# lianqi1008/Control-GIC

Hardware: AMD Instinct MI355X
Metric: encode+decode MPixels/s at fixed granularity ratio; bpp match vs reference (higher is better)
Workload: dtype f32; 1 GPU; batch 64 of 256x256 per GPU per step, codebook 1024x4, ratio (0.1,0.8,0.1), hot path only (entropy maps + router + VQ + Huffman/mask coder, encode+decode); conv encoder/decoder out of scope, latent synthetic; inputs=8 distinct resident batches in rotation (416 MiB > 256 MiB Infinity Cache)

## Files before the change

control-gic_amd/csrc/cgic_decode.hip:

```cpp
#include "cgic_coder_dev.h"

#include <atomic>

namespace cgic {

constexpr int kWinBytes = 8192;
constexpr int kWinWords = kWinBytes / 4 + 4;

struct WaveDecoder {
    const TableDev &t;
    const uint32_t *lut;
    uint32_t *win;
    const uint8_t *in;
    int nbytes;
    int wb;

    __device__ __forceinline__ void fill(int first_byte)
    {
        const int lane = lane_id();
        wb = first_byte & ~3;
        const uintptr_t g = reinterpret_cast<uintptr_t>(in) + (uintptr_t)wb;
        const uint32_t *ga = reinterpret_cast<const uint32_t *>(g & ~(uintptr_t)3);
        wsh = (int)(g & 3);
        const int limit = (nbytes - wb + wsh + 3) / 4 + 2;
// ... 572 lines not shown
        if (n0 <= 0) a.dcount[b * 3] = n0 == 0 ? -1 : -2;
        if (n1 <= 0) a.dcount[b * 3 + 1] = n1 == 0 ? -1 : -2;
        if (n2 <= 0) a.dcount[b * 3 + 2] = n2 == 0 ? -1 : -2;
    }
    if (s < 0) return;
    const int64_t n_c = (a.h >> 2) * (a.w >> 2), n_m = (a.h >> 1) * (a.w >> 1), n_f = a.h * a.w;
    const int64_t off = s == 0 ? 0 : (s == 1 ? n_c : n_c + n_m);
    const int cap = (int)(s == 0 ? n_c : (s == 1 ? n_m : n_f));
    int32_t *dc = a.dcount + b * 3 + s;
    const uint8_t *in = in0 + s * a.slot;
    const int nb = s == 0 ? n0 : s == 1 ? n1 : n2;
    const int s_pad = s == 0 ? pad0 : s == 1 ? pad1 : pad2;
    __syncthreads();
    uint16_t *dst = a.dsym + b * (n_c + n_m + n_f) + off;
    auto put = [&](int k, int sym) { dst[k] = (uint16_t)sym; };
    FastTables *ft = reinterpret_cast<FastTables *>(reinterpret_cast<int32_t *>(seg + 1) + 2 * kLdsTrieNodes);
    if (nparts == 1) {
        int nw = (nb + 15) >> 4;
        nw = nw < 1 ? 1 : (nw > kDecWaves ? kDecWaves : nw);
        if (nb <= kFastChunks * 8)
            decode_segmented<false>(a.tab, lut, win + wave * kSegWinWords, seg, in, nb, s_pad, 0, wave < nw ? nw : 0, wave, cap, put,
                                    &s_count, ft);
        else
            decode_segmented<true>(a.tab, lut, win + wave * kSegWinWords, seg, in, nb, s_pad, 0, wave < nw ? nw : 0, wave, cap, put,
                                   &s_count, ft);
        __syncthreads();
        if (tid == 0) *dc = s_count > cap ? -3 : s_count;
        return;
    }
    PartSync ps{a.bf + (b * 3 + s) * kDecPartsMax * kWave, a.tick + (b * 3 + s) * kTicketStride, s_entry};
    int nbits = s_pad == 0 ? 0 : (nb - 1) * 8 - s_pad;
    nbits = nbits < 0 ? 0 : nbits;
    const int nchunks = (nbits + kWave - 1) / kWave, per_part = (nchunks + nparts - 1) / nparts;
    if (per_part <= kFastChunks) {
        decode_segmented<true>(a.tab, lut, win + wave * kSegWinWords, seg, in, nb, s_pad, 0, kDecWaves, wave, cap, put, &s_count, ft,
                               part, nparts, 0, 0, nullptr, &ps);
    } else {
        decode_segmented<false>(a.tab, lut, win + wave * kSegWinWords, seg, in, nb, s_pad, 0, kDecWaves, wave, 0,
                                [](int, int) {}, &s_count, (FastTables *)nullptr, part, nparts, 0, 0, s_fn);
        __syncthreads();
        if (wave == 0) part_exchange(part, nparts, s_fn[tid], ps);
        if (tid == 0) s_count = 0;
        __syncthreads();
        decode_segmented<true>(a.tab, lut, win + wave * kSegWinWords, seg, in, nb, s_pad, 0, kDecWaves, wave, cap, put, &s_count, ft,
                               part, nparts, s_entry[0], s_entry[1]);
    }
    __syncthreads();
    if (tid == 0 && part == nparts - 1) *dc = s_count > cap ? -3 : s_count;
}

__global__ __launch_bounds__(kDecThreads) void decode_split_kernel(DecodeArgs a)
{
    decode_split_body(a, own_blk());
}

__global__ __launch_bounds__(kDecThreads) void decode_split_grouped_kernel(Grouped<DecodeArgs> g)
{
    Blk blk;
    decode_split_body(g.a[group_locate(g, &blk)], blk);
}

struct MergeArgs {
    const uint8_t *in;
    int64_t slot;
    const int32_t *nbytes;
    int64_t h, w;
    int mode;
    const uint16_t *dsym;
    const int32_t *dcount;
    int64_t *ind_out;
    int32_t *mc_out, *mm_out, *mf_out;
    const float *codebook;
    int K;
    float *zq;
    const float *codebook2;
    float *zq2;
    int32_t *status;
    int stage_sym, stage_cb;
    int64_t band_syms;
};

__device__ __forceinline__ void wait_decoded(unsigned int *done, unsigned int need, unsigned int total)
{
    if (threadIdx.x == 0) {
        while (__hip_atomic_load(done, __ATOMIC_RELAXED, __HIP_MEMORY_SCOPE_AGENT) < need) __builtin_amdgcn_s_sleep(8);
        const unsigned int old = __hip_atomic_fetch_add(done, 1u, __ATOMIC_RELAXED, __HIP_MEMORY_SCOPE_AGENT);
        if (old + 1u == total) __hip_atomic_store(done, 0u, __ATOMIC_RELAXED, __HIP_MEMORY_SCOPE_AGENT);
        __builtin_amdgcn_fence(__ATOMIC_ACQUIRE, "agent");
    }
    __syncthreads();
}

typedef unsigned int cgic_u32x4 __attribute__((ext_vector_type(4)));
typedef unsigned int cgic_u32x2 __attribute__((ext_vector_type(2)));
__device__ __forceinline__ void nt_store16(void *p, const void *v)
{
    __builtin_nontemporal_store(*reinterpret_cast<const cgic_u32x4 *>(v), reinterpret_cast<cgic_u32x4 *>(p));
}
__device__ __forceinline__ void nt_store8(void *p, const void *v)
{
    __builtin_nontemporal_store(*reinterpret_cast<const cgic_u32x2 *>(v), reinterpret_cast<cgic_u32x2 *>(p));
}

template <int NT, bool WAIT = false>
__device__ __forceinline__ void merge_body(const MergeArgs &a, const Blk blk, unsigned int *done = nullptr, unsigned int need = 0,
                                           unsigned int total = 0)
{
    extern __shared__ __attribute__((aligned(16))) uint32_t sm[];
    __shared__ uint32_t scan_smem[NT / kWave + 1];
    __shared__ int s_status;
    __shared__ int s_hdr[8];
    const int tid = threadIdx.x;
    const int band = blk.x;
    const int64_t b = blk.y;
    const int64_t h = a.h, w = a.w, h2 = h >> 1, w2 = w >> 1, h4 = h >> 2, w4 = w >> 2;
    const int64_t n_c = h4 * w4, n_m = h2 * w2, n_f = h * w;
    const int64_t wc = (n_c + 31) >> 5, wm = (n_m + 31) >> 5;
    const int64_t nsym = n_c + n_m + n_f;
    float4 *cbk = reinterpret_cast<float4 *>(sm);
    uint16_t *lsym = reinterpret_cast<uint16_t *>(cbk + (a.stage_cb ? a.K : 0));
    uint32_t *rawc = reinterpret_cast<uint32_t *>(lsym) + (a.stage_sym ? (nsym + 1) / 2 : 0);
    uint32_t *rawm = rawc + wc + 2;
    uint32_t *mcb = rawm + wm + 2;
    uint32_t *mmb = mcb + wc;
    uint32_t *pcb = mmb + wm;
    uint32_t *pmb = pcb + wc;
    const int mode = a.mode;
    const int64_t nbands = blk.nx;
    const int64_t rows_per = ((h4 + nbands - 1) / nbands) * 4;
    const int64_t r0 = band * rows_per, r1 = r0 + rows_per < h ? r0 + rows_per : h;
    if (r0 >= h) return;
    CGIC_STAMP(10);
    const bool send_mc = mode == 0 || mode == 2 || mode == 3;
    const bool send_mm = mode == 0 || mode == 1;
    const uint8_t *in_mc = a.in + (b * CGIC_NUM_STREAMS + 3) * a.slot;
    const uint8_t *in_mm = a.in + (b * CGIC_NUM_STREAMS + 4) * a.slot;

    if (tid == 0) s_status = 0;
    if (tid < 2) s_hdr[tid] = a.nbytes[b * CGIC_NUM_STREAMS + 3 + tid];
    else if (!WAIT && tid < 5) s_hdr[tid] = a.dcount[b * 3 + (tid - 2)];
    if (send_mc) for (int64_t i = tid; i < wc + 2; i += NT) rawc[i] = reinterpret_cast<const uint32_t *>(in_mc)[i];
    if (send_mm) for (int64_t i = tid; i < wm + 2; i += NT) rawm[i] = reinterpret_cast<const uint32_t *>(in_mm)[i];
    const uint16_t *gsym = a.dsym + b * nsym;
    if (!WAIT && a.stage_sym) {
        const uint32_t *g32 = reinterpret_cast<const uint32_t *>(gsym);
        uint32_t *l32 = reinterpret_cast<uint32_t *>(lsym);
        for (int64_t i = tid; i < (nsym + 1) / 2; i += NT) l32[i] = g32[i];
    }
    if (a.stage_cb && a.zq)
        for (int i = tid; i < a.K; i += NT) cbk[i] = reinterpret_cast<const float4 *>(a.codebook)[i];
    __syncthreads();
    CGIC_STAMP(11);

    if (tid == 0) {
        if (send_mc && (s_hdr[0] != 2 + (n_c >> 3) || (int)(rawc[0] & 0xFF) != 8 - (int)(n_c & 7))) s_status = CGIC_ERR_INVALID;
        if (send_mm && (s_hdr[1] != 2 + (n_m >> 3) || (int)(rawm[0] & 0xFF) != 8 - (int)(n_m & 7))) s_status = CGIC_ERR_INVALID;
    }
    __syncthreads();
    if (s_status) {
        if (WAIT) wait_decoded(done, need, total);
        if (tid == 0 && a.status) atomicMin(&a.status[b], s_status);
        return;
    }
    auto stream_word = [](const uint32_t *raw, int64_t wi, int64_t nbits) -> uint32_t {
        const uint64_t two = (uint64_t)raw[wi] | ((uint64_t)raw[wi + 1] << 32);
        const uint32_t pay = (uint32_t)(two >> 8);
        uint32_t v = __builtin_bswap32(__brev(pay));
        const int64_t rem = nbits - wi * 32;
        if (rem < 32) v &= rem <= 0 ? 0u : ((1u << rem) - 1u);
        return v;
    };
    uint32_t cnt_c, cnt_m;
    __shared__ uint32_t s_cnt[2];
    const bool derived_mm = mode == 3 || mode == 5;
    if (wc <= kWave && wm <= kWave && !derived_mm) {
        const int lane = lane_id(), wave = tid >> 6;
        if (wave < 2) {
            const bool co = wave == 0;
            const int64_t nw_ = co ? wc : wm, nb_ = co ? n_c : n_m;
            uint32_t v = 0;
            if (lane < nw_) {
                if (co ? send_mc : send_mm) v = stream_word(co ? rawc : rawm, lane, nb_);
                else if (co && mode == 4) {
                    v = 0xFFFFFFFFu;
                    const int64_t rem = nb_ - (int64_t)lane * 32;
                    if (rem < 32) v &= (1u << rem) - 1u;
                }
            }
            const uint32_t c = (uint32_t)__popc(v);
            const uint32_t inc = wave_inclusive_scan(c);
            if (lane < nw_) {
                (co ? mcb : mmb)[lane] = v;
                (co ? pcb : pmb)[lane] = inc - c;
            }
            if (lane == kWave - 1) s_cnt[wave] = inc;
        }
        __syncthreads();
        cnt_c = s_cnt[0];
        cnt_m = s_cnt[1];
    } else {
        for (int64_t i = tid; i < wc; i += NT) {
            uint32_t v = 0;
            if (send_mc) v = stream_word(rawc, i, n_c);
            else if (mode == 4) {
                v = 0xFFFFFFFFu;
                const int64_t rem = n_c - i * 32;
                if (rem < 32) v &= (1u << rem) - 1u;
            }
            mcb[i] = v;
        }
        __syncthreads();
        for (int64_t i = tid; i < wm; i += NT) {
            uint32_t v = 0;
            if (send_mm) v = stream_word(rawm, i, n_m);
            else if (mode == 3 || mode == 5) {
                for (int k = 0; k < 32; ++k) {
                    const int64_t j = i * 32 + k;
                    if (j >= n_m) break;
                    bool bit = true;
                    if (mode == 3) {
                        const int64_t y = j / w2, x = j - y * w2, c = (y >> 1) * w4 + (x >> 1);
                        bit = !((mcb[c >> 5] >> (c & 31)) & 1u);
                    }
                    v |= (uint32_t)bit << k;
                }
            }
            mmb[i] = v;
        }
        __syncthreads();
        if (wc <= NT && wm <= NT) {
            __shared__ unsigned long long scan64[NT / kWave + 1];
            const unsigned long long c = ((unsigned long long)(tid < wc ? __popc(mcb[tid]) : 0) << 32) | (unsigned long long)(tid < wm ? __popc(mmb[tid]) : 0);
            unsigned long long tot;
            const unsigned long long ex = block_exclusive_scan(c, scan64, &tot);
            if (tid < wc) pcb[tid] = (uint32_t)(ex >> 32);
            if (tid < wm) pmb[tid] = (uint32_t)ex;
            cnt_c = (uint32_t)(tot >> 32);
            cnt_m = (uint32_t)tot;
            __syncthreads();
        } else {
        uint32_t carry = 0, total;
        for (int64_t base = 0; base < wc; base += NT) {
            const int64_t i = base + tid;
            const uint32_t c = i < wc ? (uint32_t)__popc(mcb[i]) : 0u;
            const uint32_t ex = block_exclusive_scan(c, scan_smem, &total);
            if (i < wc) pcb[i] = carry + ex;
            carry += total;
        }
        cnt_c = carry;
        carry = 0;
        for (int64_t base = 0; base < wm; base += NT) {
            const int64_t i = base + tid;
            const uint32_t c = i < wm ? (uint32_t)__popc(mmb[i]) : 0u;
            const uint32_t ex = block_exclusive_scan(c, scan_smem, &total);
            if (i < wm) pmb[i] = carry + ex;
            carry += total;
        }
        cnt_m = carry;
        __syncthreads();
        }
    }
    CGIC_STAMP(12);

    auto fine_flag = [&](int64_t y, int64_t x, bool *pbc, bool *pbm) -> bool {
        const int64_t j2 = (y >> 1) * w2 + (x >> 1), j4 = (y >> 2) * w4 + (x >> 2);
        const bool bc = (mcb[j4 >> 5] >> (j4 & 31)) & 1u;
        const bool bm = (mmb[j2 >> 5] >> (j2 & 31)) & 1u;
        *pbc = bc; *pbm = bm;
        switch (mode) {
        case 0: return (1 - (int)bm - (int)bc) == 1;
        case 1: return !bm;
        case 2: return !bc;
        case 6: return true;
        default: return false;
        }
    };
    uint32_t fbase = 0;
    {
        uint32_t mine = 0;
        const int wvm = tid >> 6, lnm = tid & 63;
        for (int y2 = wvm; y2 < (int)(r0 >> 1); y2 += NT / 64)
            for (int x2 = lnm; x2 < (int)w2; x2 += 64) {
                bool bc, bm;
                mine += fine_flag(2 * y2, 2 * x2, &bc, &bm) ? 4u : 0u;
            }
        (void)block_exclusive_scan(mine, scan_smem, &fbase);
    }
    CGIC_STAMP(13);
    if (WAIT) {
        wait_decoded(done, need, total);
        if (tid >= 2 && tid < 5) s_hdr[tid] = a.dcount[b * 3 + (tid - 2)];
        if (a.stage_sym) {
            const uint32_t *g32 = reinterpret_cast<const uint32_t *>(gsym);
            uint32_t *l32 = reinterpret_cast<uint32_t *>(lsym);
            for (int64_t i = tid; i < (nsym + 1) / 2; i += NT) l32[i] = g32[i];
        }
        __syncthreads();
    }

    const uint16_t *ds_c = a.stage_sym ? lsym : gsym, *ds_m = ds_c + n_c, *ds_f = ds_m + n_m;
    const int64_t dc_c = s_hdr[2], dc_m = s_hdr[3], dc_f = s_hdr[4];
    uint16_t *bsym = reinterpret_cast<uint16_t *>(pmb + wm);
    int64_t off_c = 0, off_m = 0, off_f = 0;
    if (!a.stage_sym && a.band_syms > 0) {
        auto rank_of = [&](const uint32_t *bits, const uint32_t *pre, int64_t j, int64_t nbits, uint32_t total) -> int64_t {
            if (j >= nbits) return (int64_t)total;
            return (int64_t)pre[j >> 5] + __popc(bits[j >> 5] & ((1u << (j & 31)) - 1u));
        };
        const int64_t c0 = rank_of(mcb, pcb, (r0 >> 2) * w4, n_c, cnt_c), c1 = rank_of(mcb, pcb, (r1 >> 2) * w4, n_c, cnt_c);
        const int64_t m0 = rank_of(mmb, pmb, (r0 >> 1) * w2, n_m, cnt_m), m1 = rank_of(mmb, pmb, (r1 >> 1) * w2, n_m, cnt_m);
        const int64_t f0 = fbase, f1 = f0 + (r1 - r0) * w;
        const int64_t nc = c1 - c0, nm = m1 - m0, nf = (f1 < n_f ? f1 : n_f) - f0;
        if (nc >= 0 && nm >= 0 && nf >= 0 && nc + nm + nf + 3 <= a.band_syms) {
            for (int64_t i = tid; i < nc; i += NT) bsym[i] = ds_c[c0 + i];
            for (int64_t i = tid; i < nm; i += NT) bsym[nc + i] = ds_m[m0 + i];
            for (int64_t i = tid; i < nf; i += NT) bsym[nc + nm + i] = ds_f[f0 + i];
            __syncthreads();
            off_c = c0; off_m = m0 - nc; off_f = f0 - nc - nm;
            ds_c = bsym; ds_m = bsym; ds_f = bsym;
        }
    }
    const bool has_c = mode == 0 || mode == 2 || mode == 3 || mode == 4;
    const bool has_m = mode == 0 || mode == 1 || mode == 3 || mode == 5;
    const bool has_f = mode == 0 || mode == 1 || mode == 2 || mode == 6;
    int st = 0;
    if (dc_c == -3 || dc_m == -3 || dc_f == -3) st = CGIC_ERR_INVALID;
    if (has_c && dc_c >= 0 && dc_c != cnt_c) st = CGIC_ERR_INVALID;
    if (has_m && dc_m >= 0 && dc_m != cnt_m) st = CGIC_ERR_INVALID;
    const bool use_c = has_c && dc_c >= 0, use_m = has_m && dc_m >= 0, use_f = has_f && dc_f >= 0;

    int64_t *ind_out = a.ind_out ? a.ind_out + b * n_f : nullptr;
    float *zq = a.zq ? a.zq + b * 4 * n_f : nullptr;
    float *zq2 = a.zq2 ? a.zq2 + b * 4 * n_f : nullptr;
    uint32_t fcarry = fbase;
    int bad_index = 0;
    const int w4i = (int)w4;
    for (int64_t qbase = r0 * w4; qbase < r1 * w4; qbase += NT) {
        const int64_t q = qbase + tid;
        const bool live = q < r1 * w4;
        int64_t v[4] = {0, 0, 0, 0};
        bool bfa = false, bfb = false;
        int y = 0, xq = 0;
        if (live) {
            y = (int)q / w4i; xq = (int)q - y * w4i;
            const int64_t j4 = (int64_t)(y >> 2) * w4 + xq, j2 = (int64_t)(y >> 1) * w2 + 2 * xq;
            bool bc, bma, bmb, dummy;
            bfa = fine_flag(y, 4 * xq, &bc, &bma);
            bfb = fine_flag(y, 4 * xq + 2, &dummy, &bmb);
            bad_index |= (int)(mode == 0 && bc && (bma || bmb));
            int64_t vc = 0, va = 0, vb = 0;
            if (bc && use_c) vc = ds_c[(int64_t)pcb[j4 >> 5] + __popc(mcb[j4 >> 5] & ((1u << (j4 & 31)) - 1u)) - off_c];
            if (use_m) {
                const uint32_t word = mmb[j2 >> 5], below = word & ((1u << (j2 & 31)) - 1u);
                const int64_t rk = (int64_t)pmb[j2 >> 5] + __popc(below) - off_m;
                if (bma) va = ds_m[rk];
                if (bmb) vb = ds_m[rk + (bma ? 1 : 0)];
            }
            v[0] = v[1] = vc + va;
            v[2] = v[3] = vc + vb;
            const int64_t i = (int64_t)y * w + 4 * xq;
            if (a.mc_out && (y & 3) == 0) a.mc_out[b * n_c + j4] = bc;
            if (a.mm_out && (y & 1) == 0) { const int2 t2 = make_int2(bma, bmb); nt_store8(a.mm_out + b * n_m + j2, &t2); }
            if (a.mf_out) { const int4 t4 = make_int4(bfa, bfa, bfb, bfb); nt_store16(a.mf_out + b * n_f + i, &t4); }
        }
        uint32_t ftotal;
        uint32_t frank = block_exclusive_scan((bfa ? 2u : 0u) + (bfb ? 2u : 0u), scan_smem, &ftotal) + fcarry;
        if (live) {
            if (bfa) {
                if (use_f) {
                    if ((int64_t)frank < dc_f) v[0] += ds_f[(int64_t)frank - off_f];
                    if ((int64_t)frank + 1 < dc_f) v[1] += ds_f[(int64_t)frank + 1 - off_f];
                }
                frank += 2;
            }
            if (bfb && use_f) {
                if ((int64_t)frank < dc_f) v[2] += ds_f[(int64_t)frank - off_f];
                if ((int64_t)frank + 1 < dc_f) v[3] += ds_f[(int64_t)frank + 1 - off_f];
            }
            const int64_t i = (int64_t)y * w + 4 * xq;
            if (ind_out) {
                nt_store16(ind_out + i, &v[0]);
                nt_store16(ind_out + i + 2, &v[2]);
            }
            if (zq || zq2) {
#pragma unroll
                for (int k = 0; k < 4; ++k)
                    if (v[k] < 0 || v[k] >= a.K) { bad_index = 1; v[k] = 0; }
            }
            if (zq) {
                float4 e[4];
#pragma unroll
                for (int k = 0; k < 4; ++k) e[k] = a.stage_cb ? cbk[v[k]] : reinterpret_cast<const float4 *>(a.codebook)[v[k]];
                const float4 o0 = make_float4(e[0].x, e[1].x, e[2].x, e[3].x), o1 = make_float4(e[0].y, e[1].y, e[2].y, e[3].y);
                const float4 o2 = make_float4(e[0].z, e[1].z, e[2].z, e[3].z), o3 = make_float4(e[0].w, e[1].w, e[2].w, e[3].w);
                nt_store16(zq + i, &o0);
                nt_store16(zq + n_f + i, &o1);
                nt_store16(zq + 2 * n_f + i, &o2);
                nt_store16(zq + 3 * n_f + i, &o3);
            }
            if (zq2) {
                float4 e[4];
#pragma unroll
                for (int k = 0; k < 4; ++k) e[k] = reinterpret_cast<const float4 *>(a.codebook2)[v[k]];
                *reinterpret_cast<float4 *>(zq2 + i) = make_float4(e[0].x, e[1].x, e[2].x, e[3].x);
                *reinterpret_cast<float4 *>(zq2 + n_f + i) = make_float4(e[0].y, e[1].y, e[2].y, e[3].y);
                *reinterpret_cast<float4 *>(zq2 + 2 * n_f + i) = make_float4(e[0].z, e[1].z, e[2].z, e[3].z);
                *reinterpret_cast<float4 *>(zq2 + 3 * n_f + i) = make_float4(e[0].w, e[1].w, e[2].w, e[3].w);
            }
        }
        fcarry += ftotal;
    }
    CGIC_STAMP(14);
    if (r1 == h && has_f && (dc_f >= 0 ? dc_f != (int64_t)fcarry : fcarry != 0)) st = CGIC_ERR_INVALID;
    if (bad_index) s_status = CGIC_ERR_INVALID;
    __syncthreads();
    if (tid == 0 && a.status && (st || s_status)) atomicMin(&a.status[b], st ? st : s_status);
}

template <int NT>
__global__ __launch_bounds__(NT) void merge_kernel(MergeArgs a)
{
    merge_body<NT>(a, own_blk());
}

__global__ __launch_bounds__(kMergeThreads) void merge_grouped_kernel(Grouped<MergeArgs> g)
{
    Blk blk;
    merge_body<kMergeThreads>(g.a[group_locate(g, &blk)], blk);
}

struct DecodeMergeArgs {
// ... 250 lines not shown
```

control-gic_amd/csrc/cgic_decode_ss.hip:

```cpp
#include "cgic_coder_dev.h"

namespace cgic {

constexpr int kSsEnd = 0xFF;

struct SsLayout {
    int nbits[3];
    int c[4];
    int off[3];
};
__device__ __forceinline__ int sel3(int s, int v0, int v1, int v2) { return s == 0 ? v0 : (s == 1 ? v1 : v2); }

__device__ __forceinline__ uint32_t ss_bits(uint32_t d0, uint32_t d1, uint32_t d2, int pos)
{
    const uint32_t hi = pos < 32 ? d0 : d1, lo = pos < 32 ? d1 : d2;
    const uint32_t r = __builtin_amdgcn_alignbit(hi, lo, 32u - ((uint32_t)pos & 31u));
    return (pos & 31) ? r : hi;
}

template <bool WRITE, typename Put>
__device__ __forceinline__ int ss_walk(const TableDev &t, const uint32_t *lut, const uint8_t *stage, const SsLayout &L, int g,
                                       int entry, int *count, Put put)
{
    const int s = (g >= L.c[1]) + (g >= L.c[2]);
// ... 21 lines not shown
        auto step = [&]() {
            const bool go = pos < lim;
            const uint32_t e = *reinterpret_cast<const uint32_t *>(lutb + ((w0 >> ish) & imask));
            const int len = (int)(e & 0xFF);
            const int np = pos + len;
            const bool ok = go && np <= remc;
            if (WRITE) { if (ok) put(s, n, (int)(e >> 8)); }
            const uint32_t r = 32u - (uint32_t)len;
            w0 = __builtin_amdgcn_alignbit(w0, w1, r);
            w1 = __builtin_amdgcn_alignbit(w1, w2, r);
            w2 <<= (len & 31);
            pos = go ? np : pos;
            n += ok ? 1 : 0;
        };
        while (__builtin_amdgcn_ballot_w64(pos < lim) != 0) {
            step();
            step();
        }
        *count = n;
        return (pos < 64 || pos > remc) ? kSsEnd : pos - 64;
    }
    while (pos < 64) {
        if (pos >= rem) { *count = n; return kSsEnd; }
        const uint32_t bits = ss_bits(d0, d1, d2, pos);
        const uint32_t e = lut[bits >> (32 - LB)];
        int len = (int)(e & 0xFF), sym = (int)(e >> 8);
        if (len == 0) {
            if (sym == 0xFFFFFF) { *count = n; return kSsEnd; }
            const unsigned long long w0 = ((unsigned long long)d0 << 32) | d1, w1 = ((unsigned long long)d2 << 32) | d3;
            const unsigned long long win = pos ? (w0 << pos) | (w1 >> (64 - pos)) : w0;
            int node = sym, k = LB;
            sym = -1;
            while (pos + k < rem && k < 64) {
                const int c = t.child[2 * node + (int)((win >> (63 - k)) & 1ull)];
                ++k;
                if (c == INT32_MIN) break;
                if (c < 0) { sym = ~c; break; }
                node = c;
            }
            if (sym < 0) { *count = n; return kSsEnd; }
            len = k;
        }
        if (pos + len > rem) { *count = n; return kSsEnd; }
        if (WRITE) put(s, n, sym);
        pos += len;
        ++n;
    }
    *count = n;
    return pos - 64;
}


constexpr int kSsMaxSweeps = 32;
constexpr int kMeEntries = 15;
constexpr uint32_t kMeEnd = 15;

struct MeFn { uint32_t r[4]; };

__device__ __forceinline__ MeFn me_identity() { return MeFn{{0x03020100u, 0x07060504u, 0x0B0A0908u, 0x0F0E0D0Cu}}; }
__device__ __forceinline__ MeFn me_const0() { return MeFn{{0u, 0u, 0u, 0u}}; }
__device__ __forceinline__ MeFn me_compose(const MeFn &prev, const MeFn &cur)
{
    MeFn o;
#pragma unroll
    for (int k = 0; k < 4; ++k) {
        const uint32_t sel = prev.r[k];
        const uint32_t s7 = sel & 0x07070707u;
        const uint32_t lo = __builtin_amdgcn_perm(cur.r[1], cur.r[0], s7);
        const uint32_t hi = __builtin_amdgcn_perm(cur.r[3], cur.r[2], s7);
        const uint32_t m = ((sel >> 3) & 0x01010101u) * 0xFFu;
        o.r[k] = (hi & m) | (lo & ~m);
    }
    return o;
}
__device__ __forceinline__ uint32_t me_apply(const MeFn &f, uint32_t e)
{
    const uint32_t w = e < 8 ? (e < 4 ? f.r[0] : f.r[1]) : (e < 12 ? f.r[2] : f.r[3]);
    return (w >> (8 * (e & 3))) & 0xFFu;
}
__device__ __forceinline__ MeFn me_shfl_up(const MeFn &f, int d)
{
    MeFn o;
#pragma unroll
    for (int k = 0; k < 4; ++k) o.r[k] = (uint32_t)__shfl_up((int)f.r[k], d, kWave);
    return o;
}
__device__ __forceinline__ MeFn me_wave_scan(MeFn f)
{
    const int lane = lane_id();
#pragma unroll
    for (int d = 1; d < kWave; d <<= 1) {
        const MeFn p = me_shfl_up(f, d);
        const MeFn c = me_compose(p, f);
        if (lane >= d) f = c;
    }
    return f;
}

__device__ __forceinline__ MeFn me_walk_all(const TableDev &t, const uint32_t *lut, const uint8_t *stage, const SsLayout &L, int g,
                                            unsigned long long *cnt_lo, unsigned long long *cnt_hi)
{
    const int s = (g >= L.c[1]) + (g >= L.c[2]);
    const int ch = g - sel3(s, L.c[0], L.c[1], L.c[2]);
    const int rem = sel3(s, L.nbits[0], L.nbits[1], L.nbits[2]) - 64 * ch;
    const uint32_t *q = reinterpret_cast<const uint32_t *>(stage + sel3(s, L.off[0], L.off[1], L.off[2]) + 8 * ch);
    const uint32_t r0 = __builtin_bswap32(q[0]), r1 = __builtin_bswap32(q[1]), r2 = __builtin_bswap32(q[2]), r3 = __builtin_bswap32(q[3]);
    const uint32_t d0 = __builtin_amdgcn_alignbit(r0, r1, 24), d1 = __builtin_amdgcn_alignbit(r1, r2, 24), d2 = __builtin_amdgcn_alignbit(r2, r3, 24);
    const int LB = t.lut_bits;
    const int remc = rem < 128 ? rem : 128, lim = rem < 64 ? rem : 64;
    const uint32_t ish = 30u - (uint32_t)LB, imask = ((1u << LB) - 1u) << 2;
    const char *lutb = reinterpret_cast<const char *>(lut);
    const int E = t.max_len < kMeEntries ? t.max_len : kMeEntries;
    int pos[kMeEntries], n[kMeEntries];
#pragma unroll
    for (int e = 0; e < kMeEntries; ++e) { pos[e] = e < E ? e : 1 << 20; n[e] = 0; }
    for (;;) {
        bool any = false;
#pragma unroll
        for (int e = 0; e < kMeEntries; ++e) any |= pos[e] < lim;
        if (__builtin_amdgcn_ballot_w64(any) == 0) break;
#pragma unroll
        for (int e = 0; e < kMeEntries; ++e) {
            const int p = pos[e];
            const bool go = p < lim;
            const uint32_t bits = ss_bits(d0, d1, d2, p & 63);
            const uint32_t ent = *reinterpret_cast<const uint32_t *>(lutb + ((bits >> ish) & imask));
            const int np = p + (int)(ent & 0xFF);
            const bool ok = go && np <= remc;
            pos[e] = go ? np : p;
            n[e] += ok ? 1 : 0;
        }
    }
    MeFn f;
    unsigned long long lo = 0, hi = 0;
#pragma unroll
    for (int k = 0; k < 4; ++k) f.r[k] = 0;
#pragma unroll
    for (int e = 0; e < kMeEntries; ++e) {
        const int p = pos[e];
        const uint32_t x = (e >= E || p < 64 || p > remc) ? kMeEnd : (uint32_t)(p - 64);
        f.r[e >> 2] |= x << (8 * (e & 3));
        if (e < 8) lo |= (unsigned long long)(uint32_t)n[e] << (8 * e);
        else hi |= (unsigned long long)(uint32_t)n[e] << (8 * (e - 8));
    }
    f.r[3] |= kMeEnd << 24;
    *cnt_lo = lo; *cnt_hi = hi;
    return f;
}

__device__ __forceinline__ void decode_image_body(const DecodeArgs &a, const int stage_cap, const int chunk_cap, const Blk blk)
{
    extern __shared__ __attribute__((aligned(16))) uint32_t sm[];
    __shared__ int s_scan[kDecWaves + 1];
    __shared__ int s_base[4];
    __shared__ MeFn s_fn[kDecWaves];
    uint32_t *lut = sm;
    uint8_t *stage = reinterpret_cast<uint8_t *>(lut + (1 << a.tab.lut_bits));
    uint8_t *ent = stage + stage_cap, *ext = ent + chunk_cap, *cnt = ext + chunk_cap;
    const int tid = threadIdx.x, T = blockDim.x, lane = lane_id(), wave = tid >> 6, nw = T >> 6;
    const int64_t b = blk.x;
    CGIC_STAMP3(0);
    const uint8_t *in0 = a.in + (b * CGIC_NUM_STREAMS) * a.slot;
    int nb[3];
#pragma unroll
    for (int s = 0; s < 3; ++s) nb[s] = (a.stream_mask >> s & 1) ? a.nbytes[b * CGIC_NUM_STREAMS + s] : -2;
    const int pad[3] = {in0[0], in0[a.slot], in0[2 * a.slot]};
    {
        const uint4 *gl = reinterpret_cast<const uint4 *>(a.tab.lut);
        uint4 *dl = reinterpret_cast<uint4 *>(lut);
        const int n4 = (1 << a.tab.lut_bits) >> 2;
        const bool mark = a.tab.max_len <= a.tab.lut_bits;
        auto fix = [mark](uint32_t e) { return mark && (e & 0xFFu) == 0u ? e | 0xFFu : e; };
        if (n4 == 0 && tid < (1 << a.tab.lut_bits)) lut[tid] = fix(a.tab.lut[tid]);
        for (int base = 0; base < n4; base += 8 * T) {
            uint4 v[8];
#pragma unroll
            for (int k = 0; k < 8; ++k) {
                const int i = base + k * T + tid;
                v[k] = i < n4 ? gl[i] : uint4{0u, 0u, 0u, 0u};
            }
#pragma unroll
            for (int k = 0; k < 8; ++k) {
                const int i = base + k * T + tid;
                if (i < n4) dl[i] = uint4{fix(v[k].x), fix(v[k].y), fix(v[k].z), fix(v[k].w)};
            }
        }
    }
    const int64_t n_c = (a.h >> 2) * (a.w >> 2), n_m = (a.h >> 1) * (a.w >> 1), n_f = a.h * a.w;
    const int cap[3] = {(int)n_c, (int)n_m, (int)n_f};
    SsLayout L;
    int stage_used = 0;
    bool fits = true;
    L.c[0] = 0;
#pragma unroll
    for (int s = 0; s < 3; ++s) {
        if (nb[s] > a.slot) nb[s] = (int)a.slot;
        int bits = nb[s] <= 0 || pad[s] == 0 ? 0 : (nb[s] - 1) * 8 - pad[s];
        bits = bits < 0 ? 0 : bits;
        L.nbits[s] = bits;
        L.c[s + 1] = L.c[s] + ((bits + 63) >> 6);
        L.off[s] = stage_used;
        stage_used += bits ? (((bits + 7) >> 3) + 1 + 24 + 15) & ~15 : 0;
    }
    const int C = L.c[3];
    if (stage_used > stage_cap || C > chunk_cap) fits = false;
    if (tid == 0) {
        if (a.status) a.status[b] = 0;
#pragma unroll
        for (int s = 0; s < 3; ++s) {
            if (nb[s] <= 0) a.dcount[b * 3 + s] = nb[s] == 0 ? -1 : -2;
            else if (!fits) a.dcount[b * 3 + s] = -3;
        }
    }
    if (!fits) return;
    CGIC_STAMP3(1);
#pragma unroll
    for (int s = 0; s < 3; ++s) {
        if (!L.nbits[s]) continue;
        const int words = ((((L.nbits[s] + 7) >> 3) + 1 + 24 + 15) & ~15) >> 4;
        const uint4 *g = reinterpret_cast<const uint4 *>(in0 + s * a.slot);
        uint4 *d = reinterpret_cast<uint4 *>(stage + L.off[s]);
        const int lim = (int)(a.slot >> 4);
        for (int i = tid; i < words; i += T) d[i] = i < lim ? g[i] : uint4{0u, 0u, 0u, 0u};
    }
    __syncthreads();
    CGIC_STAMP3(2);
    const int R = (C + T - 1) / T;
    const int g0 = tid * R < C ? tid * R : C, g1 = g0 + R < C ? g0 + R : C;
    auto is_first = [&](int g) { return g == L.c[0] || g == L.c[1] || g == L.c[2]; };
    auto nop = [](int, int, int) {};
    int dbg_sweeps = 0;
    const bool all_entries = a.tab.max_len <= a.tab.lut_bits && a.tab.max_len <= kMeEntries;
    bool stuck = false;
    {
        int prev = 0;
        for (int g = g0; g < g1; ++g) {
            int e = prev;
            if (is_first(g)) e = 0;
            else if (g == g0) {
                const int sg = (g >= L.c[1]) + (g >= L.c[2]);
                const int chg = g - sel3(sg, L.c[0], L.c[1], L.c[2]);
                const int m = (64 * chg) % a.tab.len_gcd;
                e = m ? a.tab.len_gcd - m : 0;
            }
            int n;
            prev = ss_walk<false>(a.tab, lut, stage, L, g, e, &n, nop);
            ent[g] = (uint8_t)e; ext[g] = (uint8_t)prev; cnt[g] = (uint8_t)n;
        }
    }
    __syncthreads();
    CGIC_STAMP3(3);
    for (;;) {
        ++dbg_sweeps;
        int changed = 0;
        for (int g = g0; g < g1; ++g) {
            const int e = is_first(g) ? 0 : ext[g - 1];
            if (e != ent[g]) {
                int n;
                const int x = ss_walk<false>(a.tab, lut, stage, L, g, e, &n, nop);
                ent[g] = (uint8_t)e; ext[g] = (uint8_t)x; cnt[g] = (uint8_t)n;
                changed = 1;
            }
        }
        if (!__syncthreads_or(changed)) break;
        if (all_entries && dbg_sweeps >= kSsMaxSweeps) { stuck = true; break; }
    }
    if (stuck) {
        MeFn mine = me_identity();
        unsigned long long c_lo = 0, c_hi = 0;
        for (int g = g0; g < g1; ++g) {
            MeFn f = me_walk_all(a.tab, lut, stage, L, g, &c_lo, &c_hi);
            if (is_first(g + 1)) f = me_const0();
            mine = me_compose(mine, f);
        }
        const MeFn incl = me_wave_scan(mine);
        if (lane == kWave - 1) s_fn[wave] = incl;
        __syncthreads();
        MeFn before = me_identity();
        for (int w2 = 0; w2 < wave; ++w2) before = me_compose(before, s_fn[w2]);
        MeFn prev = me_shfl_up(incl, 1);
        if (lane == 0) prev = me_identity();
        uint32_t e = me_apply(prev, me_apply(before, 0u));
        if (g0 < g1 && is_first(g0)) e = 0;
        if (R == 1) {
            if (g0 < g1) {
                const unsigned long long cw = e < 8 ? c_lo : c_hi;
                ent[g0] = (uint8_t)(e == kMeEnd ? kSsEnd : (int)e);
                cnt[g0] = e == kMeEnd ? (uint8_t)0 : (uint8_t)((cw >> (8 * (e & 7))) & 0xFFull);
            }
        } else {
            int en = e == kMeEnd ? kSsEnd : (int)e;
            for (int g = g0; g < g1; ++g) {
                if (is_first(g)) en = 0;
                int n;
                const int x = ss_walk<false>(a.tab, lut, stage, L, g, en, &n, nop);
                ent[g] = (uint8_t)en; cnt[g] = (uint8_t)n;
                en = x;
            }
        }
        dbg_sweeps += 1;
        __syncthreads();
    }
    CGIC_STAMP3(4);
    if (a.stats && tid == 0) {
        atomicAdd(&a.stats[0], (unsigned int)dbg_sweeps);
        atomicAdd(&a.stats[1], 1u);
        atomicMax(&a.stats[2], (unsigned int)dbg_sweeps);
    }
#ifdef CGIC_PHASE_CLOCKS
    if (blk.x == 0 && tid == 0) g_phase_clk[9] = dbg_sweeps;
#endif
    int mine = 0;
    for (int g = g0; g < g1; ++g) mine += cnt[g];
    int inc = wave_inclusive_scan(mine);
    if (lane == kWave - 1) s_scan[wave] = inc;
    __syncthreads();
    if (wave == 0) {
        const int v = lane < nw ? s_scan[lane] : 0;
        const int vi = wave_inclusive_scan(v);
        if (lane < nw) s_scan[lane] = vi - v;
        if (lane == nw - 1) s_scan[kDecWaves] = vi;
    }
    __syncthreads();
    int run = s_scan[wave] + inc - mine;
    const int total = s_scan[kDecWaves];
    {
        int r = run;
        for (int g = g0; g < g1; ++g) {
            if (g == L.c[1]) s_base[1] = r;
            if (g == L.c[2]) s_base[2] = r;
            r += cnt[g];
        }
        if (tid == 0) {
            s_base[0] = 0; s_base[3] = total;
            if (L.c[2] == C) s_base[2] = total;
            if (L.c[1] == C) s_base[1] = total;
        }
    }
    __syncthreads();
    CGIC_STAMP3(5);
    uint16_t *dst = a.dsym + b * (n_c + n_m + n_f);
    for (int g = g0; g < g1; ++g) {
        const int s = (g >= L.c[1]) + (g >= L.c[2]);
        const int at = run - s_base[s];
        const int cap_s = sel3(s, cap[0], cap[1], cap[2]);
        uint16_t *dst_s = dst + sel3(s, 0, (int)n_c, (int)(n_c + n_m)) + at;
        int n;
        ss_walk<true>(a.tab, lut, stage, L, g, (int)ent[g], &n,
                      [&](int, int k, int sym) { if (at + k < cap_s) dst_s[k] = (uint16_t)sym; });
        run += n;
    }
    CGIC_STAMP3(6);
    if (tid < 3 && sel3(tid, nb[0], nb[1], nb[2]) > 0) {
        const int n = s_base[tid + 1] - s_base[tid];
        a.dcount[b * 3 + tid] = n > sel3(tid, cap[0], cap[1], cap[2]) ? -3 : n;
    }
}

__global__ __launch_bounds__(kDecThreads) void decode_image_kernel(DecodeArgs a, int stage_cap, int chunk_cap)
{
    decode_image_body(a, stage_cap, chunk_cap, own_blk());
}

__global__ __launch_bounds__(kDecThreads) void decode_image_grouped_kernel(Grouped<DecodeImageArgs> g)
{
    Blk blk;
    const DecodeImageArgs &p = g.a[group_locate(g, &blk)];
    decode_image_body(p.a, p.stage_cap, p.chunk_cap, blk);
}

}

using namespace cgic;
static GroupedRegistrar reg_decode_image(KID_DECODE_IMAGE, [](const GroupRec *const *recs, int n, hipStream_t s) {
    return launch_grouped(decode_image_grouped_kernel, "decode_image_grouped_kernel", recs[0]->block, LDS_ALWAYS, recs, n, s); });
```

Before: 129,100 MPixels/s.

## Resolve self-synchronizing Huffman chunk entries with wave shuffles instead of block sweeps

For one chunk per thread, the decoder now passes chunk exit states between lanes with shuffles. It iterates within each wave until the states converge and publishes only the wave-boundary exit through shared memory, so the number of block-wide barriers and shared-memory round trips drops. The symbol-count scan is rebuilt to need a single barrier: stream bases are computed by every thread from per-wave totals, replacing the extra scan and base passes. The kernel also issues the first LUT and stream-staging global loads early, before the layout checks, to overlap their latency. In the other decode kernel, the header check is done per thread without a barrier, and the fine-flag scan is skipped when r0 is zero. In exchange the convergence logic becomes more intricate (volatile shared flags, a cap on walks per wave) and uses more registers.

```diff
diff --git a/control-gic_amd/csrc/cgic_decode.hip b/control-gic_amd/csrc/cgic_decode.hip
--- a/control-gic_amd/csrc/cgic_decode.hip
+++ b/control-gic_amd/csrc/cgic_decode.hip
@@ -748,14 +748,12 @@
     __syncthreads();
     CGIC_STAMP(11);
 
-    if (tid == 0) {
-        if (send_mc && (s_hdr[0] != 2 + (n_c >> 3) || (int)(rawc[0] & 0xFF) != 8 - (int)(n_c & 7))) s_status = CGIC_ERR_INVALID;
-        if (send_mm && (s_hdr[1] != 2 + (n_m >> 3) || (int)(rawm[0] & 0xFF) != 8 - (int)(n_m & 7))) s_status = CGIC_ERR_INVALID;
-    }
-    __syncthreads();
-    if (s_status) {
+    bool hdr_bad = false;
+    if (send_mc && (s_hdr[0] != 2 + (n_c >> 3) || (int)(rawc[0] & 0xFF) != 8 - (int)(n_c & 7))) hdr_bad = true;
+    if (send_mm && (s_hdr[1] != 2 + (n_m >> 3) || (int)(rawm[0] & 0xFF) != 8 - (int)(n_m & 7))) hdr_bad = true;
+    if (hdr_bad) {
         if (WAIT) wait_decoded(done, need, total);
-        if (tid == 0 && a.status) atomicMin(&a.status[b], s_status);
+        if (tid == 0 && a.status) atomicMin(&a.status[b], CGIC_ERR_INVALID);
         return;
     }
     auto stream_word = [](const uint32_t *raw, int64_t wi, int64_t nbits) -> uint32_t {
@@ -872,7 +870,7 @@
         }
     };
     uint32_t fbase = 0;
-    {
+    if (r0 > 0) {
         uint32_t mine = 0;
         const int wvm = tid >> 6, lnm = tid & 63;
         for (int y2 = wvm; y2 < (int)(r0 >> 1); y2 += NT / 64)
diff --git a/control-gic_amd/csrc/cgic_decode_ss.hip b/control-gic_amd/csrc/cgic_decode_ss.hip
--- a/control-gic_amd/csrc/cgic_decode_ss.hip
+++ b/control-gic_amd/csrc/cgic_decode_ss.hip
@@ -197,7 +197,9 @@
 {
     extern __shared__ __attribute__((aligned(16))) uint32_t sm[];
     __shared__ int s_scan[kDecWaves + 1];
-    __shared__ int s_base[4];
+    __shared__ int s_at[2][2];
+    __shared__ int s_capped[2];
+    __shared__ int s_sweeps;
     __shared__ MeFn s_fn[kDecWaves];
     uint32_t *lut = sm;
     uint8_t *stage = reinterpret_cast<uint8_t *>(lut + (1 << a.tab.lut_bits));
@@ -209,27 +211,18 @@
     int nb[3];
 #pragma unroll
     for (int s = 0; s < 3; ++s) nb[s] = (a.stream_mask >> s & 1) ? a.nbytes[b * CGIC_NUM_STREAMS + s] : -2;
-    const int pad[3] = {in0[0], in0[a.slot], in0[2 * a.slot]};
-    {
-        const uint4 *gl = reinterpret_cast<const uint4 *>(a.tab.lut);
-        uint4 *dl = reinterpret_cast<uint4 *>(lut);
-        const int n4 = (1 << a.tab.lut_bits) >> 2;
-        const bool mark = a.tab.max_len <= a.tab.lut_bits;
-        auto fix = [mark](uint32_t e) { return mark && (e & 0xFFu) == 0u ? e | 0xFFu : e; };
-        if (n4 == 0 && tid < (1 << a.tab.lut_bits)) lut[tid] = fix(a.tab.lut[tid]);
-        for (int base = 0; base < n4; base += 8 * T) {
-            uint4 v[8];
-#pragma unroll
-            for (int k = 0; k < 8; ++k) {
-                const int i = base + k * T + tid;
-                v[k] = i < n4 ? gl[i] : uint4{0u, 0u, 0u, 0u};
-            }
-#pragma unroll
-            for (int k = 0; k < 8; ++k) {
-                const int i = base + k * T + tid;
-                if (i < n4) dl[i] = uint4{fix(v[k].x), fix(v[k].y), fix(v[k].z), fix(v[k].w)};
-            }
-        }
+    auto pad_of = [&](int s) { return (int)(*reinterpret_cast<const uint32_t *>(in0 + s * a.slot) & 0xFFu); };
+    const int pad[3] = {pad_of(0), pad_of(1), pad_of(2)};
+    const uint4 *gl = reinterpret_cast<const uint4 *>(a.tab.lut);
+    uint4 *dl = reinterpret_cast<uint4 *>(lut);
+    const int n4 = (1 << a.tab.lut_bits) >> 2;
+    const bool mark = a.tab.max_len <= a.tab.lut_bits;
+    auto fix = [mark](uint32_t e) { return mark && (e & 0xFFu) == 0u ? e | 0xFFu : e; };
+    uint4 v0[8];
+#pragma unroll
+    for (int k = 0; k < 8; ++k) {
+        const int i = k * T + tid;
+        v0[k] = i < n4 ? gl[i] : uint4{0u, 0u, 0u, 0u};
     }
     const int64_t n_c = (a.h >> 2) * (a.w >> 2), n_m = (a.h >> 1) * (a.w >> 1), n_f = a.h * a.w;
     const int cap[3] = {(int)n_c, (int)n_m, (int)n_f};
@@ -256,17 +249,44 @@
             if (nb[s] <= 0) a.dcount[b * 3 + s] = nb[s] == 0 ? -1 : -2;
             else if (!fits) a.dcount[b * 3 + s] = -3;
         }
+        s_capped[0] = 0; s_capped[1] = 0; s_sweeps = 0;
     }
     if (!fits) return;
     CGIC_STAMP3(1);
+    const int slot4 = (int)(a.slot >> 4);
+    uint4 u0[3];
+    int words[3];
 #pragma unroll
     for (int s = 0; s < 3; ++s) {
-        if (!L.nbits[s]) continue;
-        const int words = ((((L.nbits[s] + 7) >> 3) + 1 + 24 + 15) & ~15) >> 4;
+        words[s] = L.nbits[s] ? ((((L.nbits[s] + 7) >> 3) + 1 + 24 + 15) & ~15) >> 4 : 0;
+        const uint4 *g = reinterpret_cast<const uint4 *>(in0 + s * a.slot);
+        u0[s] = tid < words[s] && tid < slot4 ? g[tid] : uint4{0u, 0u, 0u, 0u};
+    }
+    if (n4 == 0 && tid < (1 << a.tab.lut_bits)) lut[tid] = fix(a.tab.lut[tid]);
+#pragma unroll
+    for (int k = 0; k < 8; ++k) {
+        const int i = k * T + tid;
+        if (i < n4) dl[i] = uint4{fix(v0[k].x), fix(v0[k].y), fix(v0[k].z), fix(v0[k].w)};
+    }
+    for (int base = 8 * T; base < n4; base += 8 * T) {
+        uint4 v[8];
+#pragma unroll
+        for (int k = 0; k < 8; ++k) {
+            const int i = base + k * T + tid;
+            v[k] = i < n4 ? gl[i] : uint4{0u, 0u, 0u, 0u};
+        }
+#pragma unroll
+        for (int k = 0; k < 8; ++k) {
+            const int i = base + k * T + tid;
+            if (i < n4) dl[i] = uint4{fix(v[k].x), fix(v[k].y), fix(v[k].z), fix(v[k].w)};
+        }
+    }
+#pragma unroll
+    for (int s = 0; s < 3; ++s) {
         const uint4 *g = reinterpret_cast<const uint4 *>(in0 + s * a.slot);
         uint4 *d = reinterpret_cast<uint4 *>(stage + L.off[s]);
-        const int lim = (int)(a.slot >> 4);
-        for (int i = tid; i < words; i += T) d[i] = i < lim ? g[i] : uint4{0u, 0u, 0u, 0u};
+        if (tid < words[s]) d[tid] = u0[s];
+        for (int i = tid + T; i < words[s]; i += T) d[i] = i < slot4 ? g[i] : uint4{0u, 0u, 0u, 0u};
     }
     __syncthreads();
     CGIC_STAMP3(2);
@@ -277,38 +297,76 @@
     int dbg_sweeps = 0;
     const bool all_entries = a.tab.max_len <= a.tab.lut_bits && a.tab.max_len <= kMeEntries;
     bool stuck = false;
-    {
-        int prev = 0;
-        for (int g = g0; g < g1; ++g) {
-            int e = prev;
-            if (is_first(g)) e = 0;
-            else if (g == g0) {
-                const int sg = (g >= L.c[1]) + (g >= L.c[2]);
-                const int chg = g - sel3(sg, L.c[0], L.c[1], L.c[2]);
-                const int m = (64 * chg) % a.tab.len_gcd;
-                e = m ? a.tab.len_gcd - m : 0;
-            }
-            int n;
-            prev = ss_walk<false>(a.tab, lut, stage, L, g, e, &n, nop);
-            ent[g] = (uint8_t)e; ext[g] = (uint8_t)prev; cnt[g] = (uint8_t)n;
-        }
-    }
-    __syncthreads();
-    CGIC_STAMP3(3);
-    for (;;) {
-        ++dbg_sweeps;
-        int changed = 0;
-        for (int g = g0; g < g1; ++g) {
-            const int e = is_first(g) ? 0 : ext[g - 1];
-            if (e != ent[g]) {
+    const bool own = g0 < g1;
+    int e1 = 0, x1 = kSsEnd, n1 = 0;
+    if (R == 1) {
+        const bool first = own && is_first(g0);
+        volatile uint8_t *vext = ext;
+        if (own && !first) {
+            const int sg = (g0 >= L.c[1]) + (g0 >= L.c[2]);
+            const int chg = g0 - sel3(sg, L.c[0], L.c[1], L.c[2]);
+            const int m = (64 * chg) % a.tab.len_gcd;
+            e1 = m ? a.tab.len_gcd - m : 0;
+        }
+        if (own) x1 = ss_walk<false>(a.tab, lut, stage, L, g0, e1, &n1, nop);
+        int pub = x1;
+        if (lane == kWave - 1 && own) vext[g0] = (uint8_t)x1;
+        __syncthreads();
+        CGIC_STAMP3(3);
+        int walks = 0;
+        for (int round = 0;; ++round) {
+            int changed = 0;
+            bool need;
+            for (;;) {
+                int pe = __shfl_up(x1, 1, kWave);
+                if (lane == 0 && own && g0 > 0) pe = vext[g0 - 1];
+                if (first) pe = 0;
+                need = own && pe != e1;
+                if (__builtin_amdgcn_ballot_w64(need) == 0) break;
+                if (all_entries && walks >= kSsMaxSweeps) break;
+                if (need) { x1 = ss_walk<false>(a.tab, lut, stage, L, g0, pe, &n1, nop); e1 = pe; }
+                ++walks;
+                if (lane == kWave - 1 && x1 != pub) { vext[g0] = (uint8_t)x1; pub = x1; changed = 1; }
+            }
+            if (need) s_capped[round & 1] = 1;
+            if (!__syncthreads_or(changed | (int)need)) break;
+            if (s_capped[round & 1]) { stuck = true; break; }
+        }
+        if (lane == 0) atomicMax(&s_sweeps, walks + 1);
+    } else {
+        {
+            int prev = 0;
+            for (int g = g0; g < g1; ++g) {
+                int e = prev;
+                if (is_first(g)) e = 0;
+                else if (g == g0) {
+                    const int sg = (g >= L.c[1]) + (g >= L.c[2]);
+                    const int chg = g - sel3(sg, L.c[0], L.c[1], L.c[2]);
+                    const int m = (64 * chg) % a.tab.len_gcd;
+                    e = m ? a.tab.len_gcd - m : 0;
+                }
                 int n;
-                const int x = ss_walk<false>(a.tab, lut, stage, L, g, e, &n, nop);
-                ent[g] = (uint8_t)e; ext[g] = (uint8_t)x; cnt[g] = (uint8_t)n;
-                changed = 1;
-            }
-        }
-        if (!__syncthreads_or(changed)) break;
-        if (all_entries && dbg_sweeps >= kSsMaxSweeps) { stuck = true; break; }
+                prev = ss_walk<false>(a.tab, lut, stage, L, g, e, &n, nop);
+                ent[g] = (uint8_t)e; ext[g] = (uint8_t)prev; cnt[g] = (uint8_t)n;
+            }
+        }
+        __syncthreads();
+        CGIC_STAMP3(3);
+        for (;;) {
+            ++dbg_sweeps;
+            int changed = 0;
+            for (int g = g0; g < g1; ++g) {
+                const int e = is_first(g) ? 0 : ext[g - 1];
+                if (e != ent[g]) {
+                    int n;
+                    const int x = ss_walk<false>(a.tab, lut, stage, L, g, e, &n, nop);
+                    ent[g] = (uint8_t)e; ext[g] = (uint8_t)x; cnt[g] = (uint8_t)n;
+                    changed = 1;
+                }
+            }
+            if (!__syncthreads_or(changed)) break;
+            if (all_entries && dbg_sweeps >= kSsMaxSweeps) { stuck = true; break; }
+        }
     }
     if (stuck) {
         MeFn mine = me_identity();
@@ -330,8 +388,8 @@
         if (R == 1) {
             if (g0 < g1) {
                 const unsigned long long cw = e < 8 ? c_lo : c_hi;
-                ent[g0] = (uint8_t)(e == kMeEnd ? kSsEnd : (int)e);
-                cnt[g0] = e == kMeEnd ? (uint8_t)0 : (uint8_t)((cw >> (8 * (e & 7))) & 0xFFull);
+                e1 = e == kMeEnd ? kSsEnd : (int)e;
+                n1 = e == kMeEnd ? 0 : (int)((cw >> (8 * (e & 7))) & 0xFFull);
             }
         } else {
             int en = e == kMeEnd ? kSsEnd : (int)e;
@@ -347,6 +405,29 @@
         __syncthreads();
     }
     CGIC_STAMP3(4);
+    int mine = n1;
+    if (R != 1) for (int g = g0; g < g1; ++g) mine += cnt[g];
+    const int inc = (int)wave_inclusive_scan_u32((unsigned int)mine);
+    if (lane == kWave - 1) s_scan[wave] = inc;
+    {
+        int r = inc - mine;
+        for (int g = g0; g < g1; ++g) {
+            if (g == L.c[1]) { s_at[0][0] = wave; s_at[0][1] = r; }
+            if (g == L.c[2]) { s_at[1][0] = wave; s_at[1][1] = r; }
+            r += R == 1 ? n1 : (int)cnt[g];
+        }
+    }
+    __syncthreads();
+    const int w1 = L.c[1] < C ? s_at[0][0] : nw, w2 = L.c[2] < C ? s_at[1][0] : nw;
+    int run = inc - mine, total = 0, base1 = L.c[1] < C ? s_at[0][1] : 0, base2 = L.c[2] < C ? s_at[1][1] : 0;
+    for (int k = 0; k < nw; ++k) {
+        const int t = s_scan[k];
+        run += k < wave ? t : 0;
+        base1 += k < w1 ? t : 0;
+        base2 += k < w2 ? t : 0;
+        total += t;
+    }
+    if (R == 1) dbg_sweeps = s_sweeps;
     if (a.stats && tid == 0) {
         atomicAdd(&a.stats[0], (unsigned int)dbg_sweeps);
         atomicAdd(&a.stats[1], 1u);
@@ -355,49 +436,21 @@
 #ifdef CGIC_PHASE_CLOCKS
     if (blk.x == 0 && tid == 0) g_phase_clk[9] = dbg_sweeps;
 #endif
-    int mine = 0;
-    for (int g = g0; g < g1; ++g) mine += cnt[g];
-    int inc = wave_inclusive_scan(mine);
-    if (lane == kWave - 1) s_scan[wave] = inc;
-    __syncthreads();
-    if (wave == 0) {
-        const int v = lane < nw ? s_scan[lane] : 0;
-        const int vi = wave_inclusive_scan(v);
-        if (lane < nw) s_scan[lane] = vi - v;
-        if (lane == nw - 1) s_scan[kDecWaves] = vi;
-    }
-    __syncthreads();
-    int run = s_scan[wave] + inc - mine;
-    const int total = s_scan[kDecWaves];
-    {
-        int r = run;
-        for (int g = g0; g < g1; ++g) {
-            if (g == L.c[1]) s_base[1] = r;
-            if (g == L.c[2]) s_base[2] = r;
-            r += cnt[g];
-        }
-        if (tid == 0) {
-            s_base[0] = 0; s_base[3] = total;
-            if (L.c[2] == C) s_base[2] = total;
-            if (L.c[1] == C) s_base[1] = total;
-        }
-    }
-    __syncthreads();
     CGIC_STAMP3(5);
     uint16_t *dst = a.dsym + b * (n_c + n_m + n_f);
     for (int g = g0; g < g1; ++g) {
         const int s = (g >= L.c[1]) + (g >= L.c[2]);
-        const int at = run - s_base[s];
+        const int at = run - sel3(s, 0, base1, base2);
         const int cap_s = sel3(s, cap[0], cap[1], cap[2]);
         uint16_t *dst_s = dst + sel3(s, 0, (int)n_c, (int)(n_c + n_m)) + at;
         int n;
-        ss_walk<true>(a.tab, lut, stage, L, g, (int)ent[g], &n,
+        ss_walk<true>(a.tab, lut, stage, L, g, R == 1 ? e1 : (int)ent[g], &n,
                       [&](int, int k, int sym) { if (at + k < cap_s) dst_s[k] = (uint16_t)sym; });
         run += n;
     }
     CGIC_STAMP3(6);
     if (tid < 3 && sel3(tid, nb[0], nb[1], nb[2]) > 0) {
-        const int n = s_base[tid + 1] - s_base[tid];
+        const int n = sel3(tid, base1, base2, total) - sel3(tid, 0, base1, base2);
         a.dcount[b * 3 + tid] = n > sel3(tid, cap[0], cap[1], cap[2]) ? -3 : n;
     }
 }
```

New measurement: 131,900 MPixels/s (median of 6 runs). +2.2%, better.
